# ai4ce/DiscoNet

Hardware: AMD Instinct MI355X
Metric: scenes/sec (5-agent 256x256 BEV) (higher is better)
Workload: dtype f16 hi+lo pair per value (32 bits; 22-bit significand for |x| >= 0.125, f16 exponent range, lo subnormal below: absolute floor 2^-25); conv products as split-f16 x3 MFMA, f32 accumulate; 1 GPU; DiscoNet det eval forward (--com disco), 5-agent, batch 4 per GPU, 256x256x13 BEV, no KD, sparse voxel lists -> dense -> enc -> DiscoGraph fusion -> dec -> cls/reg heads; agents=5, batch_per_gpu=4, conv_math=sp, launch=hipGraph replay, parallelism=scene-parallel x1 (no data-path collective)

## Files before the change

disconet_amd/_lib.py:

```python
import ctypes
import os
from ctypes import (POINTER, Structure, c_char_p, c_double, c_float, c_int, c_int32, c_long, c_longlong, c_size_t,
                    c_uint64, c_void_p)

_HERE = os.path.dirname(os.path.abspath(__file__))
LIB_PATH = os.environ.get("DISCONET_HIP_LIB") or os.path.join(_HERE, "libdisconet_hip.so")


class DnError(RuntimeError):
    pass


class ConvDesc(Structure):
    _fields_ = [(n, c_int32) for n in (
        "n_images", "h_in", "w_in", "c0", "c1", "up0", "c_out", "ksize", "stride", "relu",
        "ld0", "ld1", "ldo", "math")]


class PackJob(Structure):
    _fields_ = [("desc", ConvDesc), ("weight", c_void_p), ("packed", c_void_p), ("mode", c_int32), ("cin_total", c_int32),
                ("ci_first", c_int32), ("n_in", c_int32), ("wmul", c_float), ("reserved", c_int32)]


class FoldJob(Structure):
# ... 74 lines not shown
                               c_void_p, c_int, c_void_p, c_size_t, c_void_p]),
    "dn_spconv2d_pre_pair_supported": (c_int, [POINTER(ConvDesc), POINTER(ConvDesc)]),
    "dn_spconv2d_pre_pair": (c_int, [POINTER(ConvDesc), POINTER(ConvDesc), c_void_p, c_void_p, c_void_p, c_void_p, c_void_p,
                                     c_void_p, c_void_p, c_void_p, c_void_p]),
    "dn_spconv2d_dual": (c_int, [POINTER(ConvDesc), c_void_p, c_void_p, c_void_p, c_void_p, c_void_p,
                                 c_void_p, c_void_p, c_int, c_void_p]),
    "dn_spconv2d_nhwc": (c_int, [POINTER(ConvDesc), c_void_p, c_void_p, c_void_p, c_void_p, c_void_p, c_void_p, c_int,
                                 c_void_p]),
    "dn_sp_post1x1_packed_bytes": (c_size_t, []),
    "dn_sp_post1x1_pack_weights": (c_int, [c_void_p, c_int, c_int, c_float, c_void_p, c_void_p]),
    "dn_sp_post1x1_pack_heads": (c_int, [c_void_p, c_int, c_int, c_float, c_void_p, c_void_p]),
    "dn_spconv2d_post1x1": (c_int, [POINTER(ConvDesc), POINTER(Post1x1Desc)] + [c_void_p] * 8 +
                            [c_int, c_void_p, c_void_p, c_void_p]),
    "dn_spconv_force_config": (c_int, [c_int]),
    "dn_spconv_set_upmode": (c_int, [c_int]),
    "dn_decode_boxes": (c_int, [c_void_p, c_void_p, c_void_p, c_int, c_long, c_void_p, c_void_p,
                                c_void_p]),
    "dn_detect_workspace_bytes": (c_size_t, [c_int, c_long, c_int]),
    "dn_detect": (c_int, [c_void_p, c_void_p, c_void_p, c_int, c_long, c_int, c_int, c_float, c_double, c_void_p,
                          c_void_p, c_void_p, c_void_p, c_void_p, c_size_t, c_void_p]),
    "dn_ap_match_workspace_bytes": (c_size_t, [c_int, c_int, c_int, c_int]),
    "dn_ap_match": (c_int, [c_void_p, c_void_p, c_void_p, c_void_p, c_void_p, c_int, c_int, c_int, POINTER(c_double), c_int,
                            c_void_p, c_void_p, c_void_p, c_void_p, c_void_p, c_size_t, c_void_p, c_longlong, c_void_p, c_int,
                            c_int, c_void_p]),
    "dn_ap_reset": (c_int, [c_void_p, c_int, c_void_p]),
    "dn_assign_targets_workspace_bytes": (c_size_t, [c_int, c_long, c_int]),
    "dn_assign_targets": (c_int, [c_void_p, c_void_p, c_void_p, c_int, c_long, c_int, c_double, c_double, c_int, c_void_p,
                                  c_void_p, c_void_p, c_void_p, c_void_p, c_void_p, c_size_t, c_void_p]),
    "dn_warp_neighbors": (c_int, [c_void_p, c_void_p, c_void_p, c_int, c_int, c_int, c_int, c_int,
                                  c_int, c_int, c_int, c_void_p, c_void_p]),
# ... 126 lines not shown
```

disconet_amd/csrc/common.hip:

```cpp
#include "dn_internal.h"

namespace dn {
char* err_buf() {
  static thread_local char buf[512] = {0};
  return buf;
}
namespace {
typedef unsigned u32x4 __attribute__((ext_vector_type(4)));
__global__ void __launch_bounds__(256) zero_fill_kernel(unsigned char* p, size_t head, size_t vecs, size_t tail) {
  const size_t tid = blockIdx.x * (size_t)blockDim.x + threadIdx.x, stride = (size_t)gridDim.x * blockDim.x;
  if (tid < head) p[tid] = 0;
  u32x4* v = reinterpret_cast<u32x4*>(p + head);
  for (size_t i = tid; i < vecs; i += stride) v[i] = u32x4{0u, 0u, 0u, 0u};
  if (tid < tail) p[head + 16 * vecs + tid] = 0;
}
}

hipError_t zero_fill(void* ptr, size_t bytes, hipStream_t stream) {
  if (bytes == 0) return hipSuccess;
  unsigned char* p = static_cast<unsigned char*>(ptr);
  size_t head = (16 - (reinterpret_cast<size_t>(p) & 15)) & 15;
  if (head > bytes) head = bytes;
  const size_t vecs = (bytes - head) / 16, tail = bytes - head - 16 * vecs;
  const size_t want = (vecs + 255) / 256;
  const int blocks = (int)(want < 1 ? 1 : (want > 8192 ? 8192 : want));
  hipLaunchKernelGGL(zero_fill_kernel, dim3(blocks), dim3(256), 0, stream, p, head, vecs, tail);
  return hipGetLastError();
}
}

extern "C" int dn_version(void) { return 138; }

#ifndef DN_BUILD_ID
#error "build through disconet_amd/csrc/build.py (it passes -DDN_BUILD_ID)"
#endif
static const char dn_build_id_marker[] = "dn-build-id:" DN_BUILD_ID;
extern "C" const char* dn_build_id(void) { return dn_build_id_marker + 12; }

extern "C" int dn_sp_range_flags_async(unsigned* dst_device, int reset, void* stream) {
  DN_REQUIRE(dst_device != nullptr, "sp_range_flags_async: null destination");
  hipStream_t s = (hipStream_t)stream;
  if ((reset & 2) && dn::zero_fill(dst_device, sizeof(unsigned), s) != hipSuccess)
    return dn::fail(DN_ERR_LAUNCH, "sp_range_flags_async: zero fill of the destination failed");
  const bool clear = (reset & 1) != 0;
  dn::range_collect_conv_sp(dst_device, clear, s);
  dn::range_collect_conv_spq(dst_device, clear, s);
// ... 18 lines not shown
```

disconet_amd/csrc/conv_sp.hip:

```cpp
#ifndef DN_PHASE_TIMING
#define DN_PHASE_TIMING 0
#endif
#ifndef DN_SP_ABL
#define DN_SP_ABL 0
#endif
#include "dn_internal.h"
#include "sp_layout.h"
#include "sp_device.h"
#include <cstdlib>
#include <type_traits>

#if DN_PHASE_TIMING
__device__ unsigned long long g_phase_cycles[8];
extern "C" int dn_sp_phase_cycles(unsigned long long* host8, int reset) {
  if (hipDeviceSynchronize() != hipSuccess) return -1;
  if (host8 && hipMemcpyFromSymbol(host8, HIP_SYMBOL(g_phase_cycles), sizeof(unsigned long long) * 8) != hipSuccess) return -1;
  if (reset) { unsigned long long z[8] = {0}; if (hipMemcpyToSymbol(HIP_SYMBOL(g_phase_cycles), z, sizeof z) != hipSuccess) return -1; }
  return 0;
}
#endif

namespace {

constexpr int kCUs = 256;
// ... 10 lines not shown
  int up0, c_out, cog, relu;
  int ngroups;
  int tiles_x, tiles_y, total_items, xcd_order;
  int n_cb;
  float rcp_ncb, rcp_tx, rcp_ty;
  int cout_pad, wpk_bytes;
  const unsigned char* w2;
  const float* scale2;
  const float* shift2;
  float* out_b;
  int c_out2, relu2, split2, ldo_a, ldo_b, post_f32;
  int b_total;
  int stg_row;
  KSlices ks;
  size_t ks_ws_bytes;
};

struct TileCoord {
  int img, oy0, ox0, n0;
};

template <int KS, int STRIDE, int TH, int TW, int BN, int TG, int CA, int WAVES_M, int WAVES_N,
          int WTM, int WTN, int POST, int BSTAT = 0, int UPM = 0, int AHI = 0, int KSL = 0, int NB = 2>
struct SpTile {
  using P = sp::Patch<KS, STRIDE, TH, TW>;
  static constexpr int NW = WAVES_M * WAVES_N;
  static constexpr int NT = NW * 64;
  static constexpr int TAPS = KS * KS;
  static constexpr int NS = TAPS / TG;
  static constexpr int SUB = CA * TG;
  static constexpr int NPIX = P::NPIX;
  static constexpr int AQ = AHI ? 2 : 4;
  static constexpr int A_PIECES = CA * AQ * NPIX;
  static_assert(!AHI || (KS == 3 && CA == 1 && UPM == 0), "hi-only source: 3x3 layers");
  static_assert(AHI != 2 || (BSTAT != 0 && STRIDE == 1), "bit-grid source: weight-stationary stride-1 form");
  static constexpr int A_INSTR = BSTAT ? (A_PIECES + 63) / 64 : ((A_PIECES + NT - 1) / NT) * NW;
  static constexpr int A_IT = (A_INSTR + NW - 1) / NW;
  static constexpr int A_STAGE = A_INSTR * 1024;
// ... 11 lines not shown
  static constexpr int OFF_B = 2 * A_STAGE;
  static constexpr int OFF_W2 = OFF_B + NB * B_STAGE;
  static_assert(NB == 2 || (NB == 3 && KS == 3 && CA == 1 && TG == 3 && POST == 0 && BSTAT == 0 && UPM == 0 && AHI == 0 && KSL == 0),
                "three weight stages: plain streaming 3x3 tiles, three taps per step");
  static constexpr int OFF_STG = OFF_W2 + W2_BYTES;
  static constexpr int LDS_BYTES = BSTAT ? OFF_B + W2_BYTES : OFF_STG + STG_BYTES;
  static constexpr int lds_stationary(int nsteps, int stg_row) {
    return OFF_B + nsteps * B_STEP + W2_BYTES + (POST == 1 ? NW * 32 * stg_row * 4 : 0);
  }
  static constexpr int OCC_LDS = BSTAT ? (POST == 1 ? 1 : 2) : 160 * 1024 / LDS_BYTES;
  static constexpr int OCC_MAX = (WTM * WTN >= 4 || (KSL && WTM * WTN >= 2)) ? 2 : 3;
  static_assert(!KSL || (KS == 3 && CA == 1 && POST == 0 && BSTAT == 0 && UPM == 0 && AHI == 0 && WTM * WTN <= 2),
                "K slices: plain streaming 3x3 tiles with at most two accumulator tiles per wave");
  static constexpr int OCC_W = OCC_LDS < 1 ? 1 : (OCC_LDS > OCC_MAX ? OCC_MAX : OCC_LDS);
  static constexpr int WPS = (OCC_W * NW + 3) / 4;
  static_assert(TAPS % TG == 0, "tap groups must divide the taps");
  static_assert(KS == 3 || (TG == 1 && STRIDE == 1), "1x1: one tap, stride 1");
  static_assert(KS == 1 || CA == 1, "3x3: one chunk per A stage");
  static_assert(TW == 32 || TW == 16 || TW == 8, "tile width");
  static_assert(TW != 8 || (WTM == 1 && TH == 8 && WAVES_M == 2), "8-wide tiles: 2 x 1 pixel groups");
  static_assert(TW == 8 || TH == WAVES_M * WTM * RPG, "pixel tile must match the wave layout");
  static_assert(BN == WAVES_N * WTN * 32, "channel tile must match the wave layout");
  static_assert(!(STRIDE == 2 && TW == 32), "stride 2: 16- or 8-wide tiles");
  static_assert(POST != 1 || (WAVES_N == 1 && BN == 64 && TW == 32), "fused 1x1: 64 channels in one wave");
  static_assert(POST != 2 || (WAVES_N == 1 && (BN == 32 || BN == 64)), "fused block-diagonal 1x1: whole 32-channel heads per wave");
  static_assert(LDS_BYTES <= 160 * 1024, "tile does not fit the LDS");
  static_assert(!UPM || (KS == 3 && STRIDE == 1 && TG == 3 && CA == 1 && POST == 0 && BSTAT == 0 && TH == 8 && WTM == 2 &&
                         ((TW == 32 && WAVES_M == 4) || (TW == 16 && WAVES_M == 2))),
                "row-merged up-conv: 8 x 32 or 8 x 16 streaming tiles");
};

template <int KS, int STRIDE, int TH, int TW, int BN, int TG, int CA, int WAVES_M, int WAVES_N,
          int WTM, int WTN, int POST, int ABL = 0, int BSTAT = 0, int UPM = 0, int AHI = 0, int KSL = 0, int NB = 2>
__global__ void __launch_bounds__(
    (WAVES_M * WAVES_N * 64),
    (SpTile<KS, STRIDE, TH, TW, BN, TG, CA, WAVES_M, WAVES_N, WTM, WTN, POST, BSTAT, UPM, AHI, KSL, NB>::WPS))
conv_sp_kernel(const SpArgs a) {
  using T = SpTile<KS, STRIDE, TH, TW, BN, TG, CA, WAVES_M, WAVES_N, WTM, WTN, POST, BSTAT, UPM, AHI, KSL, NB>;
  using P = typename T::P;
  constexpr bool kNoB = ABL == 1 || ABL == 3 || ABL >= 5, kNoA = ABL == 2 || ABL == 3 || ABL >= 5;
  constexpr bool kNoStore = ABL == 4 || ABL == 6 || ABL == 7, kNoLds = ABL >= 5;
  constexpr bool kNoBarrier = ABL == 7;
  constexpr int NW = T::NW, NT = T::NT, NPIX = T::NPIX, TAPS = T::TAPS, NS = T::NS, SUB = T::SUB;
  constexpr int A_IT = T::A_IT, B_IT = T::B_IT;

  extern __shared__ __attribute__((aligned(16))) unsigned char smem[];
  __shared__ __attribute__((aligned(16))) float aff1_s[POST != 0 ? 4 : 1][POST != 0 ? 64 : 4];

  const int tid = threadIdx.x;
  const int lane = tid & 63;
  const int wave = tid >> 6;
  const int wave_m = wave / WAVES_N;
  const int wave_n = wave % WAVES_N;
// ... 24 lines not shown
    spi = fdivmod(spi, a.tiles_x, a.rcp_tx, tx);
    tc.img = fdivmod(spi, a.tiles_y, a.rcp_ty, ty);
    tc.ox0 = tx * TW;
    tc.oy0 = ty * TH;
    if constexpr (AHI == 2) {
      tc.n0 = __builtin_amdgcn_readfirstlane(tc.n0);
      tc.img = __builtin_amdgcn_readfirstlane(tc.img);
      tc.ox0 = __builtin_amdgcn_readfirstlane(tc.ox0);
      tc.oy0 = __builtin_amdgcn_readfirstlane(tc.oy0);
    }
    return tc;
  };

  struct Work {
    TileCoord tc;
    int sl0, sl1, j;
  };
  auto decode_work = [&](int v) {
    Work w;
    if (KSL == 0 || v < a.ks.n_whole) {
      w.tc = decode(v);
      w.sl0 = 0; w.sl1 = KSL ? a.ks.count : 1; w.j = -1;
    } else {
      w.j = v - a.ks.n_whole;
      w.sl0 = w.j & ((1 << a.ks.log2) - 1);
      w.sl1 = w.sl0 + 1;
      w.tc = decode(a.ks.n_whole + (w.j >> a.ks.log2));
    }
    return w;
  };
  auto first_group = [&](const Work& w) { return KSL ? a.ks.bound(w.sl0) : 0; };

  int a_off[WTM], b_off[WTN], prow[WTM], pcol;
  pcol = sp::tile_col<TW>(li);
#pragma unroll
// ... 127 lines not shown
      const int blk = merged ? g * 12 + st * 6 : a.c0g * 12 + (g - a.c0g) * 9 + st * 3;
      const int soff = blk * 4 * a.cout_pad * 16;
      unsigned char* base = smem + T::OFF_B + sb * T::B_STAGE + wave * 1024;
#pragma unroll
      for (int it = 0; it < B_IT; ++it)
        if (merged || it < T::B_IT_1) dma16(rsrcw, base + it * NW * 1024, voff_b[it], soff);
      return;
    }
    const int soff = ((g * CA * TAPS + st * TG) * 4 * a.cout_pad) * 16;
    unsigned char* base = smem + T::OFF_B + sb * T::B_STAGE + wave * 1024;
#pragma unroll
    for (int it = 0; it < B_IT; ++it)
      dma16(rsrcw, base + it * NW * 1024, voff_b[it], soff);
  };

  auto compute = [&](auto t0_c, auto nu_c, const unsigned char* As, const unsigned char* Bs) {
    constexpr int T0 = decltype(t0_c)::value, NU = decltype(nu_c)::value;
    half8 ah[2][WTM], al[2][WTM], bh[2][WTN], bl[2][WTN];
    auto load = [&](auto u_c) {
      constexpr int u = decltype(u_c)::value;
      constexpr int cu = (KS == 1) ? u : 0, tap = (KS == 1) ? 0 : T0 + u;
      constexpr int toff = (cu * 4 * NPIX + sp::tap_offset<KS, STRIDE, TH, TW>(tap / KS, tap % KS)) * 16;
      constexpr int s = u & 1;
      if constexpr (kNoLds) {
        const half8 k = {(_Float16)(li * 1e-3f), (_Float16)0.5f, (_Float16)-0.25f, (_Float16)lh, 0, 0, 0, 0};
#pragma unroll
        for (int wm = 0; wm < WTM; ++wm) ah[s][wm] = al[s][wm] = k;
#pragma unroll
        for (int wn = 0; wn < WTN; ++wn) bh[s][wn] = bl[s][wn] = k;
      } else {
#pragma unroll
        for (int wm = 0; wm < WTM; ++wm) {
          ah[s][wm] = *reinterpret_cast<const half8*>(As + a_off[wm] + toff);
          if constexpr (AHI == 0) al[s][wm] = *reinterpret_cast<const half8*>(As + a_off[wm] + toff + 2 * NPIX * 16);
        }
#pragma unroll
        for (int wn = 0; wn < WTN; ++wn) {
          bh[s][wn] = *reinterpret_cast<const half8*>(Bs + b_off[wn] + u * 4 * BN * 16);
          bl[s][wn] = *reinterpret_cast<const half8*>(Bs + b_off[wn] + (u * 4 + 2) * BN * 16);
        }
      }
    };
    auto mma = [&](auto u_c) {
      constexpr int s = decltype(u_c)::value & 1;
#pragma unroll
      for (int wm = 0; wm < WTM; ++wm)
#pragma unroll
        for (int k = 0; k < WTN; ++k) {
          const int wn = (wm & 1) ? WTN - 1 - k : k;
          acc[wm][wn] = __builtin_amdgcn_mfma_f32_32x32x16_f16(bl[s][wn], ah[s][wm], acc[wm][wn], 0, 0, 0);
        }
      if constexpr (AHI == 0) {
#pragma unroll
      for (int wm = 0; wm < WTM; ++wm)
#pragma unroll
        for (int k = 0; k < WTN; ++k) {
          const int wn = (wm & 1) ? WTN - 1 - k : k;
          acc[wm][wn] = __builtin_amdgcn_mfma_f32_32x32x16_f16(bh[s][wn], al[s][wm], acc[wm][wn], 0, 0, 0);
        }
      }
#pragma unroll
      for (int wm = 0; wm < WTM; ++wm)
#pragma unroll
        for (int k = 0; k < WTN; ++k) {
          const int wn = (wm & 1) ? WTN - 1 - k : k;
          acc[wm][wn] = __builtin_amdgcn_mfma_f32_32x32x16_f16(bh[s][wn], ah[s][wm], acc[wm][wn], 0, 0, 0);
        }
    };
    load(std::integral_constant<int, 0>{});
    auto body = [&](auto u_c) {
      constexpr int u = decltype(u_c)::value;
      if constexpr (u + 1 < NU) load(std::integral_constant<int, u + 1>{});
      __builtin_amdgcn_sched_barrier(0);
      mma(u_c);
      __builtin_amdgcn_sched_barrier(0);
    };
    body(std::integral_constant<int, 0>{});
    if constexpr (NU > 1) body(std::integral_constant<int, 1>{});
    if constexpr (NU > 2) body(std::integral_constant<int, 2>{});
    if constexpr (NU > 3) body(std::integral_constant<int, 3>{});
    if constexpr (NU > 4) body(std::integral_constant<int, 4>{});
    if constexpr (NU > 5) body(std::integral_constant<int, 5>{});
    if constexpr (NU > 6) body(std::integral_constant<int, 6>{});
    if constexpr (NU > 7) body(std::integral_constant<int, 7>{});
    if constexpr (NU > 8) body(std::integral_constant<int, 8>{});
    static_assert(NU <= 9, "at most 9 sub-steps per compute call");
  };

  constexpr bool kRegAffine = POST == 0;
  f32x4 sc_r[kRegAffine ? WTN : 1][4], sh_r[kRegAffine ? WTN : 1][4];
  int aff_n0 = -1;
  half8 w2h[POST == 2 ? WTN : 1][2][2], w2l[POST == 2 ? WTN : 1][2][2];
  int w2_cb[POST == 2 ? WTN : 1];
#pragma unroll
  for (int wn = 0; wn < (POST == 2 ? WTN : 1); ++wn) w2_cb[wn] = -1;
  auto load_affine = [&](int n0) {
    if (!kRegAffine || n0 == aff_n0) return;
    aff_n0 = n0;
#pragma unroll
    for (int wn = 0; wn < WTN; ++wn)
#pragma unroll
      for (int g = 0; g < 4; ++g)
// ... 146 lines not shown
              for (int e = 0; e < 4; ++e) {
                v[e] = acc2[4 * g + e] * sc[e] + sh[e];
                if (a.relu2) v[e] = fmaxf(v[e], 0.f);
              }
              if (inside && (!kNoStore || v[0] == 12345.678f)) *reinterpret_cast<f32x4*>(opx + ch) = v;
            }
          }
        }
      }
      }
    } else if constexpr (POST == 0) {
#pragma unroll
      for (int wm = 0; wm < WTM; ++wm)
#pragma unroll
        for (int wn = 0; wn < WTN; ++wn)
          store_sp_tile(acc[wm][wn], a.scale, a.shift, a.relu, tc.n0 + (wave_n * WTN + wn) * 32, a.c_out,
                        a.out, a.cog, tc.img, tc.oy0 + prow[wm], tc.ox0 + pcol, wn);
    } else {
      const unsigned char* W2 = smem + (BSTAT ? T::OFF_B + a.b_total : T::OFF_W2);
      f32x16 acc2[WTM][2];
#pragma unroll
      for (int wm = 0; wm < WTM; ++wm) {
#pragma unroll
        for (int nt = 0; nt < 2; ++nt)
#pragma unroll
          for (int r = 0; r < 16; ++r) acc2[wm][nt][r] = 0.f;
#pragma unroll
        for (int wn = 0; wn < 2; ++wn) {
          u32x2 hi[4], lo[4];
#pragma unroll
          for (int g = 0; g < 4; ++g) {
            const int co = wn * 32 + 8 * g + 4 * lh;
// ... 247 lines not shown
#pragma unroll
                for (int e = 0; e < 4; ++e) acc[wm][wn][4 * q + e] = v[e];
              }
          fold_acc();
        }
        tot_to_acc();
        epilogue(tc);
        note_range(amax, nan_seen);
      }
      return;
    }
  }

  Work cw = decode_work(item);
  cur = cw.tc;
  setup_rsrc(cur);
  setup_voff_b(cur);
  setup_voff_a(cur, first_group(cw) * CA >= a.c0g);
  int sb = 0;
  bool a_pending = true;
  int hist_a2 = 0, hist_b1 = 0, hist_a1 = 0;
  if constexpr (NB == 3) {
    issue_a(first_group(cw), 0, false);
    issue_b(first_group(cw), 0, 0, false);
    issue_b(first_group(cw), 1, 1, false);
    hist_b1 = B_IT;
  } else {
    issue_b(first_group(cw), 0, 0, false);
    issue_a(first_group(cw), 0, false);
  }

  while (true) {
    zero_acc();
    load_affine(cur.n0);
    const bool has_next = item + G < a.total_items;
    TileCoord nxt = cur;
    int ng0 = 0;
    if (has_next) {
      const Work nw = decode_work(item + G);
      nxt = nw.tc;
      ng0 = first_group(nw);
    }
    if constexpr (KSL != 0) zero_tot();
    const int g_end = KSL ? a.ks.bound(cw.sl1) : a.ngroups;

    for (int sl = cw.sl0; sl < cw.sl1; ++sl) {
    const int g_lo = KSL ? a.ks.bound(sl) : 0, g_hi = KSL ? a.ks.bound(sl + 1) : a.ngroups;
    for (int g = g_lo; g < g_hi; ++g) {
      const bool last_g = g + 1 == g_end;
      auto step = [&](auto st_c, auto merged_c) {
        constexpr int ST = decltype(st_c)::value;
        constexpr bool MERGED = decltype(merged_c)::value;
        constexpr int NSG = MERGED ? 2 : NS;
        if constexpr (NB == 3) {
          const int young = hist_a2 + hist_b1 + hist_a1;
          if (young == 0) wait_vm0();
// ... 80 lines not shown
          for (int wn = 0; wn < WTN; ++wn)
#pragma unroll
            for (int q = 0; q < 4; ++q)
              *reinterpret_cast<f32x4*>(pb + ((wm * WTN + wn) * 4 + q) * 256) =
                  f32x4{acc[wm][wn][4 * q], acc[wm][wn][4 * q + 1], acc[wm][wn][4 * q + 2], acc[wm][wn][4 * q + 3]};
      }
    } else {
      tot_to_acc();
      epilogue(cur);
      note_range(amax, nan_seen);
    }
    if (!has_next) break;
    item += G;
    if constexpr (KSL != 0) cw = decode_work(item);
    cur = nxt;
  }
}


__global__ void sp_from_nhwc_kernel(const float* __restrict__ src, unsigned char* __restrict__ dst,
                                    int c, int ld, int cg_total, long hw, long total) {
  float amax = 0.f;
  bool nan_in = false;
  for (long idx = blockIdx.x * (long)blockDim.x + threadIdx.x; idx < total;
       idx += (long)gridDim.x * blockDim.x) {
    const long px = idx % hw;
    long r = idx / hw;
    const int oct = r % 2; r /= 2;
    const int cg = r % cg_total;
    const long img = r / cg_total;
// ... 279 lines not shown
  }
  if (g_sp_force < 0 && !upm && best_blocks * (ksl && can_split ? kslices : 1) <= kCUs) best = kSpCfgs[deep_variant(best.id)];
  return best;
}

inline long ks_plan(long T, long R, int S, size_t ws_bytes, size_t bytes_per_tile) {
  if (S <= 1 || ws_bytes < bytes_per_tile) return T;
  const long full = T / R, tail = T - full * R;
  if (tail == 0) return T;
  const double cost_split = (double)full + (double)((tail * S + R - 1) / R) / S;
  if (cost_split > (double)(full + 1) - 0.2) return T;
  const long max_split = (long)(ws_bytes / bytes_per_tile);
  return tail > max_split ? T - max_split : full * R;
}

template <int KS, int STRIDE, int TH, int TW, int BN, int TG, int CA, int WAVES_M, int WAVES_N,
          int WTM, int WTN, int POST = 0, int ABL = 0, int BSTAT = 0, int UPM = 0, int AHI = 0, int KSL = 0, int NB = 2>
int launch(SpArgs& a, const dn_conv_desc& d, hipStream_t stream) {
  using T = SpTile<KS, STRIDE, TH, TW, BN, TG, CA, WAVES_M, WAVES_N, WTM, WTN, POST, BSTAT, UPM, AHI, KSL, NB>;
  auto kern = conv_sp_kernel<KS, STRIDE, TH, TW, BN, TG, CA, WAVES_M, WAVES_N, WTM, WTN, POST, ABL, BSTAT, UPM, AHI, KSL, NB>;
  const int nchunks = a.c0g + a.c1g;
  DN_REQUIRE(nchunks % CA == 0, "spconv: chunk count %d not a multiple of %d", nchunks, CA);
  a.ngroups = nchunks / CA;
  int lds_bytes = T::LDS_BYTES;
  constexpr int kStaticLds = POST != 0 ? 1024 : 0;
  if (BSTAT) {
    a.b_total = a.ngroups * T::NS * T::B_STEP;
    a.stg_row = a.c_out2 + 4;
    lds_bytes = T::lds_stationary(a.ngroups * T::NS, a.post_f32 ? a.stg_row : 0);
    DN_REQUIRE(lds_bytes <= 160 * 1024 - kStaticLds && (d.c_out <= BN || POST == 2),
               "spconv: layer does not fit the weight-stationary form");
  }
  static dn::PerDeviceFlag attr_flag;
  bool& attr_set = attr_flag.here();
  if (!attr_set) {
// ... 5 lines not shown
                      hipGetErrorString(e));
    attr_set = true;
  }
  int occupancy = 160 * 1024 / lds_bytes;
  occupancy = occupancy < 1 ? 1 : (occupancy > T::OCC_W ? T::OCC_W : occupancy);
  a.tiles_x = (a.w_out + TW - 1) / TW;
  a.tiles_y = (a.h_out + TH - 1) / TH;
  const long total = (long)a.n_images * a.tiles_y * a.tiles_x * ((d.c_out + BN - 1) / BN);
  DN_REQUIRE(total < (1L << 31), "spconv: too many tiles (%ld)", total);
  DN_REQUIRE(total < (1L << 22), "spconv: too many work items for the reciprocal decode (%ld)", total);
  a.total_items = (int)total;
  a.xcd_order = 1;
  a.n_cb = (d.c_out + BN - 1) / BN;
  a.rcp_ncb = 1.0f / (float)a.n_cb; a.rcp_tx = 1.0f / (float)a.tiles_x; a.rcp_ty = 1.0f / (float)a.tiles_y;
  const long resident = (long)occupancy * kCUs;
  if constexpr (KSL != 0) {
    const int S = a.ks.count;
    DN_REQUIRE(S == 2 || S == 4, "spconv: %d K slices (1, 2 or 4)", S);
    DN_REQUIRE(a.ngroups >= S, "spconv: %d K slices of a %d-chunk layer", S, a.ngroups);
    KSlices& k = a.ks;
    k.count = S; k.log2 = S == 4 ? 2 : 1; k.ngroups = a.ngroups;
    k.b1 = a.ngroups / S; k.b2 = 2 * a.ngroups / S; k.b3 = 3 * a.ngroups / S;
    if (S == 2) { k.b2 = k.b3 = a.ngroups; }
    const size_t per_tile = (size_t)S * T::NW * WTM * WTN * 16 * 64 * sizeof(float);
    k.n_whole = (int)ks_plan(total, resident, S, k.partial ? a.ks_ws_bytes : 0, per_tile);
    k.n_split = (int)(total - k.n_whole);
    k.fixup = 0;
    const long work = k.n_whole + (long)k.n_split * S;
    a.total_items = (int)work;
    hipLaunchKernelGGL(kern, dim3((unsigned)(work > resident ? resident : work)), dim3(T::NT), lds_bytes, stream, a);
    if (k.n_split) {
      k.fixup = 1;
      a.total_items = k.n_split;
      hipLaunchKernelGGL(kern, dim3((unsigned)(k.n_split > 4 * kCUs ? 4 * kCUs : k.n_split)), dim3(T::NT), 0, stream, a);
    }
    return dn::check_launch("conv_sp_kernel (K slices)");
  }
  dim3 grid((unsigned)(total > resident ? resident : total));
  hipLaunchKernelGGL(kern, grid, dim3(T::NT), lds_bytes, stream, a);
  return dn::check_launch("conv_sp_kernel");
}

inline bool fits_stationary(const dn_conv_desc& d, int bn, int a_stage, int extra, int wgs,
                            bool any_blocks = false) {
  if (d.ksize != 3 || d.stride != 1 || (d.c_out > bn && !any_blocks)) return false;
  const int nchunks = chunks_of(d.c0) + chunks_of(d.c1);
  const int bytes = 2 * a_stage + nchunks * 9 * 4 * bn * 16 + extra;
  return bytes * wgs <= 160 * 1024;
}

int fill_args(const dn_conv_desc* d, const void* src0, const void* src1, const void* packed,
              const float* scale, const float* shift, void* out, SpArgs& a) {
  a.src0 = (const unsigned char*)src0; a.src1 = (const unsigned char*)src1;
  a.wpk = (const unsigned char*)packed; a.scale = scale; a.shift = shift; a.out = (unsigned char*)out;
  a.n_images = d->n_images; a.h_in = d->h_in; a.w_in = d->w_in;
  a.h_out = out_dim(d->h_in, d->ksize, d->stride);
  a.w_out = out_dim(d->w_in, d->ksize, d->stride);
  a.c0g = chunks_of(d->c0); a.c1g = chunks_of(d->c1);
  a.up0 = d->up0; a.c_out = d->c_out; a.cog = chunks_of(d->c_out); a.relu = d->relu;
  a.cout_pad = cout_pad_of(d->c_out);
  a.wpk_bytes = (int)(packed_blocks(*d) * 4 * a.cout_pad * 16);
  DN_REQUIRE((long)a.h_out * a.w_out * 16 * 4 * (a.cog > 4 ? a.cog : 4) < (1L << 31),
             "spconv: one output image of %d x %d x %d channels exceeds 2 GiB", a.h_out, a.w_out, d->c_out);
  a.w2 = nullptr; a.scale2 = nullptr; a.shift2 = nullptr; a.out_b = nullptr;
  a.c_out2 = 0; a.relu2 = 0; a.split2 = 0; a.ldo_a = 0; a.ldo_b = 0; a.post_f32 = 0;
  a.b_total = 0; a.stg_row = 0;
  a.ks = KSlices{nullptr, 1, 0, 0, 0, 0, 0, 0, 0, 0};
  a.ks_ws_bytes = 0;
  auto aligned16 = [](const void* p) { return (reinterpret_cast<uintptr_t>(p) & 15) == 0; };
  DN_REQUIRE(aligned16(src0) && aligned16(src1) && aligned16(packed) && aligned16(out),
             "spconv: tensors must be 16-byte aligned");
  return DN_OK;
}

}

namespace dn { void range_collect_conv_sp(unsigned* dst, bool reset, hipStream_t s) { sp_range_collect_here(dst, reset, s); } }
namespace dn {
unsigned* sp_range_word() {
  void* p = nullptr;
  return hipGetSymbolAddress(&p, HIP_SYMBOL(g_sp_range_flags)) == hipSuccess ? (unsigned*)p : nullptr;
}
}
// ... 137 lines not shown
extern "C" int dn_sp_post1x1_pack_heads(const float* w2, int c_out2, int split, float wmul, void* packed,
                                        void* stream) {
  DN_REQUIRE(w2 && packed, "sp heads pack: null pointer");
  DN_REQUIRE(split > 0 && split < c_out2 && split <= 64 && c_out2 - split <= 64,
             "sp heads pack: split %d of %d outputs", split, c_out2);
  hipLaunchKernelGGL(sp_pack_heads_kernel, dim3(2), dim3(256), 0, (hipStream_t)stream, w2,
                     (unsigned char*)packed, c_out2, split, wmul);
  return dn::check_launch("sp_pack_heads_kernel");
}

extern "C" int dn_spconv_force_config(int cfg) {
  g_sp_force = cfg;
  return DN_OK;
}

extern "C" int dn_spconv_set_upmode(int mode) {
  g_sp_upmode = mode;
  return DN_OK;
}

namespace {
int spconv2d_impl(const dn_conv_desc* d, const void* src0, const void* src1, const void* packed, const float* scale,
                  const float* shift, void* out, float* out_nhwc, int ld_nhwc, void* stream, int kslices = 1,
                  void* workspace = nullptr, size_t workspace_bytes = 0);
}

extern "C" int dn_spconv2d(const dn_conv_desc* d, const void* src0, const void* src1,
                           const void* packed, const float* scale, const float* shift, void* out,
                           void* stream) {
  return spconv2d_impl(d, src0, src1, packed, scale, shift, out, nullptr, 0, stream);
// ... 222 lines not shown
```

disconet_amd/csrc/sp_device.h:

```cpp
#pragma once
#include <hip/hip_runtime.h>

typedef float f32x16 __attribute__((ext_vector_type(16)));
#ifndef DN_F32X4_DEFINED
#define DN_F32X4_DEFINED
typedef float f32x4 __attribute__((ext_vector_type(4)));
#endif
typedef _Float16 half8 __attribute__((ext_vector_type(8)));
typedef _Float16 half4 __attribute__((ext_vector_type(4)));
typedef unsigned u32x2 __attribute__((ext_vector_type(2)));
typedef unsigned u32x4 __attribute__((ext_vector_type(4)));

namespace {

__device__ inline void wait_vm0() { asm volatile("s_waitcnt vmcnt(0)" ::: "memory"); }
template <int N>
__device__ inline void wait_vm() {
  static_assert(N >= 0 && N < 64, "vmcnt immediate");
  asm volatile("s_waitcnt vmcnt(%0)" ::"n"(N) : "memory");
}

__device__ inline int fdivmod(int x, int d, float rcp, int& rem) {
  int q = (int)((float)x * rcp);
  int r = x - q * d;
// ... 64 lines not shown
  return f32x4{a[0], a[1], b[0], b[1]};
}
__device__ inline f32x4 quad_of(const f32x16& c, int g) { return f32x4{c[4 * g], c[4 * g + 1], c[4 * g + 2], c[4 * g + 3]}; }

struct KSlices {
  float* partial;
  int count, log2;
  int b1, b2, b3;
  int ngroups;
  int n_whole;
  int n_split;
  int fixup;
  __host__ __device__ int bound(int s) const { return s <= 0 ? 0 : s == 1 ? b1 : s == 2 ? b2 : s == 3 ? b3 : ngroups; }
};

__device__ inline u32x4 gather_octet(u32x2 x, u32x2 y) {
  const auto s0 = __builtin_amdgcn_permlane32_swap(x[0], y[0], false, false);
  const auto s1 = __builtin_amdgcn_permlane32_swap(x[1], y[1], false, false);
  return u32x4{s0[0], s1[0], s0[1], s1[1]};
}

}
```

disconet_amd/ops.py:

```python
import ctypes
import os

import torch

from . import _lib
from ._lib import ConvDesc, FuseMlpParams, MlpTailParams, Post1x1Desc, check


def _ptr(t):
    return ctypes.c_void_p(t.data_ptr()) if t is not None else None


def _stream_handle():
    return torch._C._cuda_getCurrentRawStream(torch._C._cuda_getDevice())


def _stream():
    return ctypes.c_void_p(_stream_handle())


def _need_gpu(*tensors):
    for t in tensors:
        if t is not None and not t.is_cuda:
            raise _lib.DnError("disconet_amd ops need tensors on the MI355X (got a %s tensor); "
# ... 413 lines not shown
        check(lib.dn_spconv2d_ks(ctypes.byref(d), kslices, _ptr(src0.data), p1, _ptr(packed), _ptr(scale), _ptr(shift),
                                 _ptr(out.data), _ptr(flat), d.c_out if nhwc_copy else 0, _ptr(ws) if nbytes else None, nbytes,
                                 _stream()),
              "dn_spconv2d_ks")
        return (out, flat) if nhwc_copy else out
    if nhwc_copy:
        check(lib.dn_spconv2d_dual(ctypes.byref(d), _ptr(src0.data), p1, _ptr(packed), _ptr(scale), _ptr(shift),
                                   _ptr(out.data), _ptr(flat), d.c_out, _stream()), "dn_spconv2d_dual")
        return out, flat
    check(_lib.load().dn_spconv2d(ctypes.byref(d), _ptr(src0.data), _ptr(src1.data) if src1 is not None else None,
                                  _ptr(packed), _ptr(scale), _ptr(shift), _ptr(out.data), _stream()),
          "dn_spconv2d")
    return out


def sp_conv2d_nhwc(d, src0, packed, scale, shift, out, src1=None):
    _need_gpu(src0, packed, scale, shift, src1, out)
    ho, wo = conv_out_hw(d)
    if (tuple(out.shape) != (d.n_images, ho, wo, d.c_out) or out.dtype != torch.float32 or out.stride(3) != 1
            or out.stride(1) != wo * out.stride(2) or out.stride(0) != ho * out.stride(1)):
        raise _lib.DnError("sp_conv2d_nhwc: out must be float32 [n, h_out, w_out, c_out] rows (a channel slice is fine)")
    if src0.hi_only or src0.bits or (src1 is not None and (src1.hi_only or src1.bits)):
        raise _lib.DnError("sp_conv2d_nhwc: full SP sources only")
    check(_lib.load().dn_spconv2d_nhwc(ctypes.byref(d), _ptr(src0.data), _ptr(src1.data) if src1 is not None else None,
                                       _ptr(packed), _ptr(scale), _ptr(shift), _ptr(out), out.stride(2), _stream()),
          "dn_spconv2d_nhwc")
    return out


def sp_conv2d_pre_pair_supported(d1, d2):
# ... 236 lines not shown
```

include/disconet_hip.h:

```cpp
#ifndef DISCONET_HIP_H
#define DISCONET_HIP_H

#include <stddef.h>
#include <stdint.h>

#ifdef __cplusplus
extern "C" {
#endif

#define DN_OK 0
#define DN_ERR_ARG (-1)
#define DN_ERR_LAUNCH (-2)
#define DN_ERR_UNSUPPORTED (-3)

int dn_version(void);
const char* dn_build_id(void);
const char* dn_last_error(void);

unsigned dn_sp_range_flags(int reset);
int dn_sp_range_flags_async(unsigned* dst_device, int reset, void* stream);

int dn_voxelize_occupy(const float* pts, int n_pts, int pt_stride,
                       const double* voxel_size_host, const double* extents_host,
                       const int* dims_host, float* dense, void* stream);
// ... 90 lines not shown
                     const float* scale, const float* shift, void* out_sp, float* out_nhwc, int ld_nhwc,
                     void* stream);
int dn_spconv2d_nhwc(const dn_conv_desc* d, const void* src0_sp, const void* src1_sp, const void* packed,
                     const float* scale, const float* shift, float* out_nhwc, int ld_nhwc, void* stream);
size_t dn_sp_post1x1_packed_bytes(void);
int dn_sp_post1x1_pack_weights(const float* w2, int c_out2, int c_in2, float wmul, void* packed,
                               void* stream);
int dn_sp_post1x1_pack_heads(const float* w2, int c_out2, int split, float wmul, void* packed,
                             void* stream);
int dn_spconv2d_post1x1(const dn_conv_desc* d, const dn_post1x1_desc* p, const void* src0_sp,
                        const void* src1_sp, const void* packed, const float* scale,
                        const float* shift, const void* packed2, const float* scale2,
                        const float* shift2, int out_f32, void* out_a, float* out_b, void* stream);
int dn_spconv_force_config(int cfg);
int dn_spconv_set_upmode(int mode);

int dn_warp_neighbors(const float* feat, const float* trans, const int32_t* num_agent,
                      int batch, int agents, int h, int w, int c, int only_v2i,
                      int ego_first, int ego_count, float* warped, void* stream);

typedef struct dn_mlp_tail_params {
  const float* bn1_scale; const float* bn1_shift;
  const float* w2; const float* s2; const float* t2;
  const float* w3; const float* s3; const float* t3;
  const float* w4; const float* b4;
} dn_mlp_tail_params;

int dn_disco_fuse_tail(const float* feat, const float* warped, const float* g,
                       const float* fw, const int32_t* num_agent,
                       const dn_mlp_tail_params* p, int batch, int agents, int hw, int c,
// ... 56 lines not shown
```

Measured before the change: 2340 scenes/s.

## Split tail-wave conv tiles into half-tile work items to balance the last wave

Adds a pixel-split mode to the persistent sparse-precision conv kernel. When the tile count leaves a partial last wave across CUs, the leftover tiles are each split into two items, each computing one MFMA pixel-row half, so more workgroups share the tail. A host-side planner picks the split from tile count, resident slots and a per-shape utilization estimate, with an env/API override. The cost is duplicated A/B loads for split tiles and an extra template instantiation.

```diff
diff --git a/disconet_amd/_lib.py b/disconet_amd/_lib.py
--- a/disconet_amd/_lib.py
+++ b/disconet_amd/_lib.py
@@ -112,6 +112,8 @@
                             [c_int, c_void_p, c_void_p, c_void_p]),
     "dn_spconv_force_config": (c_int, [c_int]),
     "dn_spconv_set_upmode": (c_int, [c_int]),
+    "dn_spconv_set_psplit": (c_int, [c_int]),
+    "dn_spconv_psplit_last_plan": (c_int, [ctypes.POINTER(c_int), ctypes.POINTER(c_int)]),
     "dn_decode_boxes": (c_int, [c_void_p, c_void_p, c_void_p, c_int, c_long, c_void_p, c_void_p,
                                 c_void_p]),
     "dn_detect_workspace_bytes": (c_size_t, [c_int, c_long, c_int]),
diff --git a/disconet_amd/csrc/common.hip b/disconet_amd/csrc/common.hip
--- a/disconet_amd/csrc/common.hip
+++ b/disconet_amd/csrc/common.hip
@@ -29,7 +29,7 @@
 }
 }
 
-extern "C" int dn_version(void) { return 138; }
+extern "C" int dn_version(void) { return 139; }
 
 #ifndef DN_BUILD_ID
 #error "build through disconet_amd/csrc/build.py (it passes -DDN_BUILD_ID)"
diff --git a/disconet_amd/csrc/conv_sp.hip b/disconet_amd/csrc/conv_sp.hip
--- a/disconet_amd/csrc/conv_sp.hip
+++ b/disconet_amd/csrc/conv_sp.hip
@@ -48,6 +48,7 @@
   int stg_row;
   KSlices ks;
   size_t ks_ws_bytes;
+  PSplit ps;
 };
 
 struct TileCoord {
@@ -55,7 +56,7 @@
 };
 
 template <int KS, int STRIDE, int TH, int TW, int BN, int TG, int CA, int WAVES_M, int WAVES_N,
-          int WTM, int WTN, int POST, int BSTAT = 0, int UPM = 0, int AHI = 0, int KSL = 0, int NB = 2>
+          int WTM, int WTN, int POST, int BSTAT = 0, int UPM = 0, int AHI = 0, int KSL = 0, int NB = 2, int PSP = 0>
 struct SpTile {
   using P = sp::Patch<KS, STRIDE, TH, TW>;
   static constexpr int NW = WAVES_M * WAVES_N;
@@ -97,6 +98,8 @@
                 "K slices: plain streaming 3x3 tiles with at most two accumulator tiles per wave");
   static constexpr int OCC_W = OCC_LDS < 1 ? 1 : (OCC_LDS > OCC_MAX ? OCC_MAX : OCC_LDS);
   static constexpr int WPS = (OCC_W * NW + 3) / 4;
+  static_assert(!PSP || (POST == 0 && BSTAT == 0 && UPM == 0 && AHI == 0 && KSL == 0 && (WTM == 2 || (WTM == 1 && WAVES_M == 2))),
+                "pixel split: plain streaming tiles of two MFMA pixel-tile rows per wave or per workgroup");
   static_assert(TAPS % TG == 0, "tap groups must divide the taps");
   static_assert(KS == 3 || (TG == 1 && STRIDE == 1), "1x1: one tap, stride 1");
   static_assert(KS == 1 || CA == 1, "3x3: one chunk per A stage");
@@ -114,12 +117,12 @@
 };
 
 template <int KS, int STRIDE, int TH, int TW, int BN, int TG, int CA, int WAVES_M, int WAVES_N,
-          int WTM, int WTN, int POST, int ABL = 0, int BSTAT = 0, int UPM = 0, int AHI = 0, int KSL = 0, int NB = 2>
+          int WTM, int WTN, int POST, int ABL = 0, int BSTAT = 0, int UPM = 0, int AHI = 0, int KSL = 0, int NB = 2, int PSP = 0>
 __global__ void __launch_bounds__(
     (WAVES_M * WAVES_N * 64),
-    (SpTile<KS, STRIDE, TH, TW, BN, TG, CA, WAVES_M, WAVES_N, WTM, WTN, POST, BSTAT, UPM, AHI, KSL, NB>::WPS))
+    (SpTile<KS, STRIDE, TH, TW, BN, TG, CA, WAVES_M, WAVES_N, WTM, WTN, POST, BSTAT, UPM, AHI, KSL, NB, PSP>::WPS))
 conv_sp_kernel(const SpArgs a) {
-  using T = SpTile<KS, STRIDE, TH, TW, BN, TG, CA, WAVES_M, WAVES_N, WTM, WTN, POST, BSTAT, UPM, AHI, KSL, NB>;
+  using T = SpTile<KS, STRIDE, TH, TW, BN, TG, CA, WAVES_M, WAVES_N, WTM, WTN, POST, BSTAT, UPM, AHI, KSL, NB, PSP>;
   using P = typename T::P;
   constexpr bool kNoB = ABL == 1 || ABL == 3 || ABL >= 5, kNoA = ABL == 2 || ABL == 3 || ABL >= 5;
   constexpr bool kNoStore = ABL == 4 || ABL == 6 || ABL == 7, kNoLds = ABL >= 5;
@@ -174,11 +177,17 @@
 
   struct Work {
     TileCoord tc;
-    int sl0, sl1, j;
+    int sl0, sl1, j, part;
   };
   auto decode_work = [&](int v) {
     Work w;
-    if (KSL == 0 || v < a.ks.n_whole) {
+    w.part = -1;
+    if (PSP != 0 && v >= a.ps.n_whole) {
+      int t;
+      a.ps.item(v, t, w.part);
+      w.tc = decode(t);
+      w.sl0 = 0; w.sl1 = 1; w.j = -1;
+    } else if (KSL == 0 || v < a.ks.n_whole) {
       w.tc = decode(v);
       w.sl0 = 0; w.sl1 = KSL ? a.ks.count : 1; w.j = -1;
     } else {
@@ -336,9 +345,20 @@
       dma16(rsrcw, base + it * NW * 1024, voff_b[it], soff);
   };
 
-  auto compute = [&](auto t0_c, auto nu_c, const unsigned char* As, const unsigned char* Bs) {
-    constexpr int T0 = decltype(t0_c)::value, NU = decltype(nu_c)::value;
+  int part = -1;
+  const int wave_m_u = PSP != 0 ? __builtin_amdgcn_readfirstlane(wave) / WAVES_N : 0;
+  auto in_part = [&](int wm) { return PSP == 0 || part < 0 || (WTM == 2 ? wm == 0 : wave_m_u == part); };
+  auto set_part = [&](int p) { part = p; };
+  auto prow_of = [&](int wm) { return (PSP != 0 && WTM == 2 && part == 1) ? prow[WTM - 1] : prow[wm]; };
+  using AllWm = std::integral_constant<int, (1 << WTM) - 1>;
+
+  auto compute_wm = [&](auto wms_c, auto t0_c, auto nu_c, const unsigned char* As, const unsigned char* Bs) {
+    constexpr int T0 = decltype(t0_c)::value, NU = decltype(nu_c)::value, WMS = decltype(wms_c)::value;
     half8 ah[2][WTM], al[2][WTM], bh[2][WTN], bl[2][WTN];
+    int ao[WTM];
+#pragma unroll
+    for (int wm = 0; wm < WTM; ++wm) ao[wm] = a_off[wm];
+    if constexpr (PSP != 0 && WTM == 2 && WMS == 1) ao[0] = part == 1 ? a_off[WTM - 1] : a_off[0];
     auto load = [&](auto u_c) {
       constexpr int u = decltype(u_c)::value;
       constexpr int cu = (KS == 1) ? u : 0, tap = (KS == 1) ? 0 : T0 + u;
@@ -353,8 +373,9 @@
       } else {
 #pragma unroll
         for (int wm = 0; wm < WTM; ++wm) {
-          ah[s][wm] = *reinterpret_cast<const half8*>(As + a_off[wm] + toff);
-          if constexpr (AHI == 0) al[s][wm] = *reinterpret_cast<const half8*>(As + a_off[wm] + toff + 2 * NPIX * 16);
+          if (!((WMS >> wm) & 1)) continue;
+          ah[s][wm] = *reinterpret_cast<const half8*>(As + ao[wm] + toff);
+          if constexpr (AHI == 0) al[s][wm] = *reinterpret_cast<const half8*>(As + ao[wm] + toff + 2 * NPIX * 16);
         }
 #pragma unroll
         for (int wn = 0; wn < WTN; ++wn) {
@@ -369,6 +390,7 @@
       for (int wm = 0; wm < WTM; ++wm)
 #pragma unroll
         for (int k = 0; k < WTN; ++k) {
+          if (!((WMS >> wm) & 1)) continue;
           const int wn = (wm & 1) ? WTN - 1 - k : k;
           acc[wm][wn] = __builtin_amdgcn_mfma_f32_32x32x16_f16(bl[s][wn], ah[s][wm], acc[wm][wn], 0, 0, 0);
         }
@@ -377,6 +399,7 @@
       for (int wm = 0; wm < WTM; ++wm)
 #pragma unroll
         for (int k = 0; k < WTN; ++k) {
+          if (!((WMS >> wm) & 1)) continue;
           const int wn = (wm & 1) ? WTN - 1 - k : k;
           acc[wm][wn] = __builtin_amdgcn_mfma_f32_32x32x16_f16(bh[s][wn], al[s][wm], acc[wm][wn], 0, 0, 0);
         }
@@ -385,6 +408,7 @@
       for (int wm = 0; wm < WTM; ++wm)
 #pragma unroll
         for (int k = 0; k < WTN; ++k) {
+          if (!((WMS >> wm) & 1)) continue;
           const int wn = (wm & 1) ? WTN - 1 - k : k;
           acc[wm][wn] = __builtin_amdgcn_mfma_f32_32x32x16_f16(bh[s][wn], ah[s][wm], acc[wm][wn], 0, 0, 0);
         }
@@ -408,6 +432,19 @@
     if constexpr (NU > 8) body(std::integral_constant<int, 8>{});
     static_assert(NU <= 9, "at most 9 sub-steps per compute call");
   };
+  auto compute = [&](auto t0_c, auto nu_c, const unsigned char* As, const unsigned char* Bs) {
+    if constexpr (PSP == 0) {
+      compute_wm(AllWm{}, t0_c, nu_c, As, Bs);
+    } else {
+      if (part < 0) {
+        compute_wm(AllWm{}, t0_c, nu_c, As, Bs);
+      } else if constexpr (WTM == 2) {
+        compute_wm(std::integral_constant<int, 1>{}, t0_c, nu_c, As, Bs);
+      } else {
+        if (wave_m_u == part) compute_wm(AllWm{}, t0_c, nu_c, As, Bs);
+      }
+    }
+  };
 
   constexpr bool kRegAffine = POST == 0;
   f32x4 sc_r[kRegAffine ? WTN : 1][4], sh_r[kRegAffine ? WTN : 1][4];
@@ -584,8 +621,9 @@
       for (int wm = 0; wm < WTM; ++wm)
 #pragma unroll
         for (int wn = 0; wn < WTN; ++wn)
+          if (in_part(wm))
           store_sp_tile(acc[wm][wn], a.scale, a.shift, a.relu, tc.n0 + (wave_n * WTN + wn) * 32, a.c_out,
-                        a.out, a.cog, tc.img, tc.oy0 + prow[wm], tc.ox0 + pcol, wn);
+                        a.out, a.cog, tc.img, tc.oy0 + prow_of(wm), tc.ox0 + pcol, wn);
     } else {
       const unsigned char* W2 = smem + (BSTAT ? T::OFF_B + a.b_total : T::OFF_W2);
       f32x16 acc2[WTM][2];
@@ -863,6 +901,7 @@
 
   Work cw = decode_work(item);
   cur = cw.tc;
+  set_part(cw.part);
   setup_rsrc(cur);
   setup_voff_b(cur);
   setup_voff_a(cur, first_group(cw) * CA >= a.c0g);
@@ -885,10 +924,12 @@
     const bool has_next = item + G < a.total_items;
     TileCoord nxt = cur;
     int ng0 = 0;
+    int npart = -1;
     if (has_next) {
       const Work nw = decode_work(item + G);
       nxt = nw.tc;
       ng0 = first_group(nw);
+      npart = nw.part;
     }
     if constexpr (KSL != 0) zero_tot();
     const int g_end = KSL ? a.ks.bound(cw.sl1) : a.ngroups;
@@ -999,6 +1040,7 @@
     item += G;
     if constexpr (KSL != 0) cw = decode_work(item);
     cur = nxt;
+    set_part(npart);
   }
 }
 
@@ -1308,11 +1350,25 @@
   return tail > max_split ? T - max_split : full * R;
 }
 
+constexpr float kPsRhoMax = 0.94f;
+inline long ps_plan(long T, long R, long C, float rho) {
+  if (T < C || T >= R || !(rho <= kPsRhoMax)) return T;
+  const long n_whole = T / C * C, tail = T - n_whole;
+  if (tail == 0 || n_whole + 2 * tail > R) return T;
+  return n_whole;
+}
+template <int KS, int STRIDE, int TW, int WTM>
+constexpr float ps_rho() {
+  return (KS == 3 && STRIDE == 1 && TW == 16 && WTM == 2) ? 0.88f : 1.f;
+}
+int g_ps_mode = [] { const char* e = getenv("DN_SP_PSPLIT"); return e ? atoi(e) : -1; }();
+int g_ps_last[2] = {0, 0};
+
 template <int KS, int STRIDE, int TH, int TW, int BN, int TG, int CA, int WAVES_M, int WAVES_N,
-          int WTM, int WTN, int POST = 0, int ABL = 0, int BSTAT = 0, int UPM = 0, int AHI = 0, int KSL = 0, int NB = 2>
+          int WTM, int WTN, int POST = 0, int ABL = 0, int BSTAT = 0, int UPM = 0, int AHI = 0, int KSL = 0, int NB = 2, int PSP = 0>
 int launch(SpArgs& a, const dn_conv_desc& d, hipStream_t stream) {
-  using T = SpTile<KS, STRIDE, TH, TW, BN, TG, CA, WAVES_M, WAVES_N, WTM, WTN, POST, BSTAT, UPM, AHI, KSL, NB>;
-  auto kern = conv_sp_kernel<KS, STRIDE, TH, TW, BN, TG, CA, WAVES_M, WAVES_N, WTM, WTN, POST, ABL, BSTAT, UPM, AHI, KSL, NB>;
+  using T = SpTile<KS, STRIDE, TH, TW, BN, TG, CA, WAVES_M, WAVES_N, WTM, WTN, POST, BSTAT, UPM, AHI, KSL, NB, PSP>;
+  auto kern = conv_sp_kernel<KS, STRIDE, TH, TW, BN, TG, CA, WAVES_M, WAVES_N, WTM, WTN, POST, ABL, BSTAT, UPM, AHI, KSL, NB, PSP>;
   const int nchunks = a.c0g + a.c1g;
   DN_REQUIRE(nchunks % CA == 0, "spconv: chunk count %d not a multiple of %d", nchunks, CA);
   a.ngroups = nchunks / CA;
@@ -1348,6 +1404,7 @@
   a.n_cb = (d.c_out + BN - 1) / BN;
   a.rcp_ncb = 1.0f / (float)a.n_cb; a.rcp_tx = 1.0f / (float)a.tiles_x; a.rcp_ty = 1.0f / (float)a.tiles_y;
   const long resident = (long)occupancy * kCUs;
+  if constexpr (PSP == 0) { g_ps_last[0] = (int)total; g_ps_last[1] = 0; }
   if constexpr (KSL != 0) {
     const int S = a.ks.count;
     DN_REQUIRE(S == 2 || S == 4, "spconv: %d K slices (1, 2 or 4)", S);
@@ -1370,9 +1427,23 @@
     }
     return dn::check_launch("conv_sp_kernel (K slices)");
   }
-  dim3 grid((unsigned)(total > resident ? resident : total));
+  constexpr bool kPsForm = PSP == 0 && POST == 0 && ABL == 0 && BSTAT == 0 && UPM == 0 && AHI == 0 && KSL == 0 && TG != 9 &&
+                           TH == 8 && BN <= 64 && WTM * WTN < 4;
+  if constexpr (kPsForm) {
+    long n_whole = total;
+    if (g_ps_mode > 0) n_whole = total > g_ps_mode ? total - g_ps_mode : 0;
+    else if (g_ps_mode < 0) n_whole = ps_plan(total, resident, kCUs, ps_rho<KS, STRIDE, TW, WTM>());
+    g_ps_last[0] = (int)n_whole; g_ps_last[1] = (int)(total - n_whole);
+    if (n_whole < total) {
+      a.ps = PSplit{(int)n_whole, (int)(total - n_whole)};
+      return launch<KS, STRIDE, TH, TW, BN, TG, CA, WAVES_M, WAVES_N, WTM, WTN, POST, ABL, BSTAT, UPM, AHI, KSL, NB, 1>(a, d, stream);
+    }
+  }
+  const long items = PSP ? a.ps.items() : total;
+  a.total_items = (int)items;
+  dim3 grid((unsigned)(items > resident ? resident : items));
   hipLaunchKernelGGL(kern, grid, dim3(T::NT), lds_bytes, stream, a);
-  return dn::check_launch("conv_sp_kernel");
+  return dn::check_launch(PSP ? "conv_sp_kernel (pixel split)" : "conv_sp_kernel");
 }
 
 inline bool fits_stationary(const dn_conv_desc& d, int bn, int a_stage, int extra, int wgs,
@@ -1401,6 +1472,7 @@
   a.b_total = 0; a.stg_row = 0;
   a.ks = KSlices{nullptr, 1, 0, 0, 0, 0, 0, 0, 0, 0};
   a.ks_ws_bytes = 0;
+  a.ps = PSplit{0, 0};
   auto aligned16 = [](const void* p) { return (reinterpret_cast<uintptr_t>(p) & 15) == 0; };
   DN_REQUIRE(aligned16(src0) && aligned16(src1) && aligned16(packed) && aligned16(out),
              "spconv: tensors must be 16-byte aligned");
@@ -1568,6 +1640,17 @@
   return DN_OK;
 }
 
+extern "C" int dn_spconv_set_psplit(int mode) {
+  g_ps_mode = mode < 0 ? -1 : mode;
+  return DN_OK;
+}
+
+extern "C" int dn_spconv_psplit_last_plan(int* n_whole, int* n_split) {
+  DN_REQUIRE(n_whole && n_split, "spconv psplit: null pointer");
+  *n_whole = g_ps_last[0]; *n_split = g_ps_last[1];
+  return DN_OK;
+}
+
 extern "C" int dn_spconv_set_upmode(int mode) {
   g_sp_upmode = mode;
   return DN_OK;
diff --git a/disconet_amd/csrc/sp_device.h b/disconet_amd/csrc/sp_device.h
--- a/disconet_amd/csrc/sp_device.h
+++ b/disconet_amd/csrc/sp_device.h
@@ -102,6 +102,22 @@
   __host__ __device__ int bound(int s) const { return s <= 0 ? 0 : s == 1 ? b1 : s == 2 ? b2 : s == 3 ? b3 : ngroups; }
 };
 
+struct PSplit {
+  int n_whole;
+  int n_split;
+  __host__ __device__ int items() const { return n_whole + 2 * n_split; }
+  __host__ __device__ void item(int v, int& tile, int& part) const {
+    const int j = v - n_whole, full = n_split & ~7;
+    if (j < 2 * full) {
+      tile = n_whole + ((j >> 4) << 3) + (j & 7);
+      part = (j >> 3) & 1;
+    } else {
+      tile = n_whole + full + ((j - 2 * full) >> 1);
+      part = j & 1;
+    }
+  }
+};
+
 __device__ inline u32x4 gather_octet(u32x2 x, u32x2 y) {
   const auto s0 = __builtin_amdgcn_permlane32_swap(x[0], y[0], false, false);
   const auto s1 = __builtin_amdgcn_permlane32_swap(x[1], y[1], false, false);
diff --git a/disconet_amd/ops.py b/disconet_amd/ops.py
--- a/disconet_amd/ops.py
+++ b/disconet_amd/ops.py
@@ -451,6 +451,16 @@
     return out
 
 
+def sp_set_psplit(mode):
+    check(_lib.load().dn_spconv_set_psplit(int(mode)), "dn_spconv_set_psplit")
+
+
+def sp_psplit_last_plan():
+    n_whole, n_split = ctypes.c_int(0), ctypes.c_int(0)
+    check(_lib.load().dn_spconv_psplit_last_plan(ctypes.byref(n_whole), ctypes.byref(n_split)), "dn_spconv_psplit_last_plan")
+    return n_whole.value, n_split.value
+
+
 def sp_conv2d_nhwc(d, src0, packed, scale, shift, out, src1=None):
     _need_gpu(src0, packed, scale, shift, src1, out)
     ho, wo = conv_out_hw(d)
diff --git a/include/disconet_hip.h b/include/disconet_hip.h
--- a/include/disconet_hip.h
+++ b/include/disconet_hip.h
@@ -128,6 +128,8 @@
                         const float* shift2, int out_f32, void* out_a, float* out_b, void* stream);
 int dn_spconv_force_config(int cfg);
 int dn_spconv_set_upmode(int mode);
+int dn_spconv_set_psplit(int mode);
+int dn_spconv_psplit_last_plan(int* n_whole, int* n_split);
 
 int dn_warp_neighbors(const float* feat, const float* trans, const int32_t* num_agent,
                       int batch, int agents, int h, int w, int c, int only_v2i,
```

Result: no change. 2341 scenes/s (median of 2 runs) (+0.0%).
